# yinyajun/Details-In-Recommendation

Hardware: AMD Instinct MI355X
Metric: CTR samples/sec (embedding gather + FM 2nd-order, 26-field batch 65536) (higher is better)
Workload: dtype f32; 1 GPU; deepfm_gather_fm; batch=65536, fields=26, vocab_per_field=1000000, dim=16, ids=uniform, id_layout=bf, row_policy=auto, parallelism=single GPU, tables resident (1.66 GB)

## Files before the change

### details-in-recommendation_amd/_lib.py

```python
import ctypes
import os

_HERE = os.path.dirname(os.path.abspath(__file__))
_LIB_PATH = os.environ.get("DIR_HIP_LIBRARY") or os.path.join(_HERE, "libdir_hip.so")

c_i32, c_i64, c_f32p, c_vp = ctypes.c_int, ctypes.c_int64, ctypes.c_void_p, ctypes.c_void_p

SIGNATURES = {
    "dir_version": (c_i32, []),
    "dir_last_error": (ctypes.c_char_p, []),
    "dir_crc32c": (ctypes.c_uint32, [ctypes.c_uint32, c_vp, c_i64]),
    "dir_embedding_bag_f32": (c_i32, [c_vp, c_i32, c_i32, c_vp, c_vp, c_vp, c_i64, c_i64, c_i32, c_i32, c_i64,
                                      c_vp, c_i64, c_vp]),
    "dir_embedding_bag_ex_f32": (c_i32, [c_vp, c_vp, c_i32, c_i32, c_vp, c_vp, c_vp, c_i64, c_i64, c_vp, c_i32, ctypes.c_float, c_i32,
                                         c_i64, c_vp, c_i64, c_vp]),
    "dir_embedding_bag_ex2_f32": (c_i32, [c_vp, c_vp, c_i32, c_i32, c_vp, c_vp, c_vp, c_i64, c_i64, c_vp, c_i32, c_vp, ctypes.c_float, c_i32,
                                          c_i64, c_vp, c_i64, c_vp]),
    "dir_check_ids": (c_i32, [c_vp, c_i32, c_vp, c_vp, c_i64, c_i64, c_i64, c_vp, c_vp]),
    "dir_fm_second_order_f32": (c_i32, [c_vp, c_i64, c_i64, c_i32, c_i32, c_vp, c_vp]),
    "dir_linear_onehot_rows_f32": (c_i32, [c_vp, c_i64, c_vp, c_i32, c_vp, c_i64, c_i64, c_vp, c_i32, c_i64, c_vp, c_vp]),
    "dir_sparse_ftrl_rows_sorted_f32": (c_i32, [c_vp, c_i32, c_vp, c_i64, c_i64, c_vp, c_i64, c_i64, ctypes.c_float, ctypes.c_float,
                                                ctypes.c_float, c_i64, c_vp, c_i64, c_vp, c_i64, c_vp, c_vp]),
    "dir_gather_fm_fused_f32": (c_i32, [c_vp, c_vp, c_i32, c_i32, c_vp, c_i64, c_i64, c_i32, c_i64, c_vp, c_i64, c_vp, c_vp]),
    "dir_gather_fm_linear_packed_f32": (c_i32, [c_vp, c_vp, c_i32, c_i32, c_i64, c_i32, c_vp, c_i64, c_i64, c_i32, c_i64, c_vp, c_i64,
                                                c_vp, c_vp, c_vp, c_vp]),
    "dir_gather_fm_rows_f32": (c_i32, [c_vp, c_vp, c_i32, c_i32, c_i64, c_vp, c_i64, c_i64, c_i32, c_i64, c_vp, c_i64, c_vp, c_vp, c_vp]),
    "dir_gather_fm_rows_bits_f32": (c_i32, [c_vp, c_vp, c_i32, c_i32, c_i64, c_vp, c_i64, c_i64, c_i32, c_i64, c_vp, c_i64, c_vp, c_vp, c_vp,
                                            c_vp, c_vp, c_vp]),
    "dir_linear_sparse_sum_f32": (c_i32, [c_vp, c_vp, c_i32, c_vp, c_vp, c_vp, c_i64, c_i64, c_i32, c_vp, c_i32, c_i64,
                                          c_vp, c_vp]),
    "dir_dcn_cross_f32": (c_i32, [c_vp, c_i64, c_vp, c_vp, c_i32, c_i64, c_i32, c_vp, c_i64, c_vp]),
    "dir_dcn_cross_op_f32": (c_i32, [c_vp, c_vp, c_i64, c_vp, c_vp, c_i64, c_i32, c_vp, c_i64, c_vp]),
    "dir_dcn_cross_head_f32": (c_i32, [c_vp, c_i64, c_vp, c_vp, c_i32, c_i64, c_i32, c_vp, c_vp, c_i64, c_vp, c_vp]),
    "dir_fm_second_order_backward_f32": (c_i32, [c_vp, c_i64, c_vp, c_vp, c_i64, c_i64, c_i32, c_i32, c_vp, c_i64, c_vp]),
    "dir_dense_gated_f32": (c_i32, [c_vp, c_i64, c_vp, c_i64, c_vp, c_i64, c_i64, c_i32, c_i32, c_vp, c_i64, c_vp]),
    "dir_dense_dw_bf16x3_workspace_bytes": (c_i64, [c_i64, c_i32, c_i32]),
    "dir_dense_dw_bf16x3_f32": (c_i32, [c_vp, c_i64, c_vp, c_i64, c_i64, c_i32, c_i32, c_vp, c_i64, c_vp, c_vp, c_i64, c_vp]),
    "dir_dense_dw_f16x2_f32": (c_i32, [c_vp, c_i64, c_vp, c_i64, c_i64, c_i32, c_i32, c_vp, c_i64, c_vp, c_vp, c_i64, c_vp, c_vp]),
    "dir_dense_dw_f16x2_scaled_f32": (c_i32, [c_vp, c_i64, c_vp, c_i64, c_i64, c_i32, c_i32, c_vp, c_i64, c_vp, c_vp, c_i64, c_vp, c_vp, c_vp]),
    "dir_row_absmax_workspace_words": (c_i32, []),
    "dir_row_absmax_bits_f32": (c_i32, [c_vp, c_i64, c_i64, c_i32, c_vp, c_vp, c_vp, c_vp]),
    "dir_dense_f16x2_rows_f32": (c_i32, [c_vp, c_i64, c_vp, c_vp, c_i32, c_vp, c_vp, c_vp, c_i64, c_i64, c_i32, c_i32, c_vp, c_i64, c_vp, c_vp, c_vp, c_vp]),
    "dir_dense_dw_small_workspace_bytes": (c_i64, [c_i64, c_i32, c_i32]),
    "dir_dense_dw_small_f32": (c_i32, [c_vp, c_i64, c_vp, c_i64, c_i64, c_i32, c_i32, c_vp, c_i64, c_vp, c_vp, c_i64, c_vp]),
    "dir_units1_relu_backward_partials": (c_i64, [c_i64, c_i32]),
    "dir_units1_relu_backward_f32": (c_i32, [c_vp, c_vp, c_vp, c_i64, c_i64, c_i32, c_vp, c_i64, c_vp, c_i64, c_vp]),
    "dir_units1_relu_backward_bits_f32": (c_i32, [c_vp, c_vp, c_vp, c_i64, c_i64, c_i32, c_vp, c_i64, c_vp, c_i64, c_vp, c_vp, c_vp]),
    "dir_units1_backward_partials": (c_i64, [c_i64, c_i32]),
    "dir_units1_backward_f32": (c_i32, [c_vp, c_vp, c_vp, c_i64, c_i64, c_i32, c_vp, c_i64, c_vp, c_vp, c_i64, c_vp]),
    "dir_units1_f32": (c_i32, [c_vp, c_i64, c_i64, c_i32, c_vp, c_vp, c_vp, c_i64, c_vp]),
    "dir_bn_train_partials": (c_i64, [c_i64, c_i32]),
    "dir_bn_train_stats_f32": (c_i32, [c_vp, c_i64, c_i64, c_i32, ctypes.c_float, ctypes.c_float, c_vp, c_vp, c_vp, c_vp, c_vp, c_vp, c_vp, c_vp, c_vp,
                                       c_i64, c_vp]),
    "dir_bn_train_backward_f32": (c_i32, [c_vp, c_i64, c_vp, c_i64, c_i64, c_i32, c_vp, c_vp, c_vp, c_i32, c_vp, c_i64, c_vp, c_vp, c_vp, c_vp, c_i64,
                                          c_vp]),
    "dir_dice_train_backward_f32": (c_i32, [c_vp, c_i64, c_vp, c_i64, c_i64, c_i32, c_vp, c_vp, c_vp, c_vp, c_vp, c_vp, c_i64, c_vp, c_vp, c_vp, c_i64,
                                            c_vp]),
    "dir_dense_affine_f32": (c_i32, [c_vp, c_i64, c_vp, c_i64, c_vp, c_i32, c_vp, c_vp, c_i64, c_i32, c_i32, c_vp, c_i64, c_vp]),
    "dir_dense_small_f32": (c_i32, [c_vp, c_i64, c_vp, c_i64, c_vp, c_i32, c_vp, c_vp, c_i64, c_i32, c_i32, c_vp, c_i64, c_vp]),
    "dir_dense_mid_f32": (c_i32, [c_vp, c_i64, c_vp, c_i64, c_vp, c_i32, c_vp, c_vp, c_i64, c_i32, c_i32, c_vp, c_i64, c_vp]),
    "dir_tower_bf16x3_image_bytes": (c_i64, [c_i32, c_i32]),
    "dir_tower_bf16x3_pack_f32": (c_i32, [c_vp, c_i64, c_i32, c_i32, c_vp, c_i64, c_vp]),
    "dir_tower_bf16x3_f32": (c_i32, [c_vp, c_i64, c_i64, c_i32, c_i32, c_vp, c_vp, c_vp, c_vp, c_vp, c_vp, c_vp, c_vp, c_vp, c_vp, c_vp, c_i64, c_vp]),
    "dir_deepfm_tower_bf16x3_f32": (c_i32, [c_vp, c_vp, c_i32, c_i32, c_i64, c_i32, c_vp, c_i64, c_i64, c_i32, c_i64, c_vp, c_i32, c_vp, c_vp, c_vp, c_vp,
                                            c_vp, c_vp, c_vp, c_vp, c_vp, c_vp, c_vp, c_i64, c_vp]),
    "dir_tower_f16x2_pack_f32": (c_i32, [c_vp, c_i64, c_i32, c_i32, c_vp, c_i64, c_vp]),
    "dir_tower_f16x2_f32": (c_i32, [c_vp, c_i64, c_i64, c_i32, c_i32, c_vp, c_vp, c_vp, c_vp, c_vp, c_vp, c_vp, c_vp, c_vp, c_vp, c_vp, c_i64, c_vp]),
    "dir_deepfm_tower_f16x2_f32": (c_i32, [c_vp, c_vp, c_i32, c_i32, c_i64, c_i32, c_vp, c_i64, c_i64, c_i32, c_i64, c_vp, c_i32, c_vp, c_vp, c_vp, c_vp,
                                           c_vp, c_vp, c_vp, c_vp, c_vp, c_vp, c_vp, c_i64, c_vp]),
    "dir_esmm_head_f32": (c_i32, [c_vp, c_vp, c_i64, ctypes.c_float, c_vp, c_vp]),
    "dir_tower_cs_image_bytes": (c_i64, [c_i32, c_i32]),
    "dir_tower_cs_f16x2_pack_f32": (c_i32, [c_vp, c_i64, c_i32, c_i32, c_vp, c_i64, c_vp]),
    "dir_tower_cs_f16x2_f32": (c_i32, [c_vp, c_i64, c_i64, c_i32, c_i32, c_vp, c_vp, c_vp, c_vp, c_vp, c_vp, c_vp, c_vp, c_vp, c_vp, c_vp, c_i64, c_vp]),
    "dir_deepfm_tower_cs_f16x2_f32": (c_i32, [c_vp, c_vp, c_i32, c_i32, c_i64, c_i32, c_vp, c_i64, c_i64, c_i32, c_i64, c_vp, c_i32, c_vp, c_vp, c_vp, c_vp,
                                              c_vp, c_vp, c_vp, c_vp, c_vp, c_vp, c_vp, c_i64, c_vp]),
    "dir_dense_f16x2_pack_strided_f32": (c_i32, [c_vp, c_i64, c_i64, c_i32, c_i32, c_vp, c_i64, c_vp]),
# ... 217 lines not shown
```

### details-in-recommendation_amd/csrc/embedding_bag.hip

```cpp
#include "common.hpp"
#include "bag_row.hpp"

namespace dir {

template <int LPS, int VEC, int KT, int UF, bool DO_FM, bool DO_OUT, bool NT>
__global__ __launch_bounds__(256) void gather_onehot_k(const float* const* __restrict__ tables,
                                                       const int64_t* __restrict__ vocab,
                                                       const int64_t* __restrict__ ids, int64_t sb,
                                                       int64_t sf, int F, int Krt, int64_t B,
                                                       float* __restrict__ out, int64_t out_ld,
                                                       float* __restrict__ fm) {
    using V = typename VecT<VEC>::T;
    constexpr int SPW = 64 / LPS;
    const int K = KT > 0 ? KT : Krt;
    const int lane = threadIdx.x & 63;
    const int c = lane & (LPS - 1);
    const int s = lane / LPS;
    const int kv = (K + VEC - 1) / VEC;
    const bool cact = c < kv;
    const int64_t nwave = (int64_t)gridDim.x * (blockDim.x >> 6);
    for (int64_t g = (int64_t)blockIdx.x * (blockDim.x >> 6) + (threadIdx.x >> 6); g * SPW < B; g += nwave) {
        const int64_t b = g * SPW + s;
        const bool act = cact && (b < B);
        const int64_t* idp = ids + (act ? b * sb : 0);
        float* op = DO_OUT ? out + (act ? b * out_ld : 0) + c * VEC : nullptr;
        V sum = vzero((V*)nullptr), sq = vzero((V*)nullptr);
        for (int f0 = 0; f0 < F; f0 += UF) {
            int64_t id[UF];
#pragma unroll
            for (int u = 0; u < UF; ++u) {
                const int f = f0 + u;
                id[u] = (act && f < F) ? idp[(int64_t)f * sf] : (int64_t)-1;
            }
            V row[UF];
#pragma unroll
            for (int u = 0; u < UF; ++u) {
                const int f = f0 + u;
                row[u] = vzero((V*)nullptr);
                if (f < F) {
                    const float* t = tables[f];
                    if ((uint64_t)id[u] < id_bound(vocab, f)) row[u] = NT ? ldv_nt(t + id[u] * K + c * VEC, (V*)nullptr) : ldv(t + id[u] * K + c * VEC, (V*)nullptr);
                }
            }
#pragma unroll
            for (int u = 0; u < UF; ++u) {
                const int f = f0 + u;
                if (f < F) {
                    if (DO_OUT && act) stv(op + (int64_t)f * K, row[u]);
                    if (DO_FM) {
                        sum = vadd(sum, row[u]);
                        sq = vadd(sq, vmul(row[u], row[u]));
                    }
                }
            }
        }
        if (DO_FM) {
            float r = fm_tail<LPS>(sum, sq, lane, c);
            if (c == LPS - 1 && b < B) fm[b] = r;
        }
    }
}

template <int LPS, int UF, bool NT>
__global__ __launch_bounds__(256) void gather_packed_rows_k(const float* const* __restrict__ tables,
                                                            const int64_t* __restrict__ vocab,
                                                            const int64_t* __restrict__ ids, int64_t sb, int64_t sf,
                                                            int F, int K, int64_t ld, int lin_col, int64_t B,
                                                            float* __restrict__ out, int64_t out_ld,
                                                            float* __restrict__ fm, const float* __restrict__ bias,
                                                            float* __restrict__ lin_out,
                                                            float* __restrict__ fsum ,
                                                            unsigned int* __restrict__ row_bits = nullptr ,
                                                            unsigned int* __restrict__ all_bits = nullptr ,
                                                            unsigned int* __restrict__ block_bits = nullptr, unsigned int* __restrict__ ticket = nullptr) {
// ... 184 lines not shown
                                            int K, float* __restrict__ out) {
    using V = typename VecT<VEC>::T;
    constexpr int SPW = 64 / LPS;
    const int lane = threadIdx.x & 63;
    const int c = lane & (LPS - 1);
    const int s = lane / LPS;
    const int kv = (K + VEC - 1) / VEC;
    const bool cact = c < kv;
    const int64_t nwave = (int64_t)gridDim.x * (blockDim.x >> 6);
    for (int64_t g = (int64_t)blockIdx.x * (blockDim.x >> 6) + (threadIdx.x >> 6); g * SPW < B; g += nwave) {
        const int64_t b = g * SPW + s;
        const bool act = cact && (b < B);
        const float* ep = emb + (act ? b * ld : 0) + c * VEC;
        V sum = vzero((V*)nullptr), sq = vzero((V*)nullptr);
#pragma unroll 8
        for (int f = 0; f < F; ++f) {
            V r = act ? ldv(ep + (int64_t)f * K, (V*)nullptr) : vzero((V*)nullptr);
            sum = vadd(sum, r);
            sq = vadd(sq, vmul(r, r));
        }
        float r = fm_tail<LPS>(sum, sq, lane, c);
        if (c == LPS - 1 && b < B) out[b] = r;
    }
}

__global__ void check_ids_k(const int64_t* __restrict__ vocab, int F, const int64_t* __restrict__ ids,
                            const int64_t* __restrict__ offsets, int64_t sb, int64_t sf, int64_t B,
                            int32_t* __restrict__ bad) {
    const int64_t n = B * F;
    int local = 0;
    for (int64_t i = (int64_t)blockIdx.x * blockDim.x + threadIdx.x; i < n; i += (int64_t)gridDim.x * blockDim.x) {
        const int64_t b = i / F;
        const int f = (int)(i - b * F);
        const int64_t v = vocab[f];
        if (!offsets) {
            const int64_t id = ids[b * sb + f * sf];
            if (id >= v || id < -1) ++local;
        } else {
            const int64_t bag = b * sb + f * sf;
            for (int64_t e = offsets[bag]; e < offsets[bag + 1]; ++e)
                if (ids[e] >= v || ids[e] < -1) ++local;
        }
    }
    if (local) atomicAdd(bad, local);
}

static int next_pow2(int v) {
    int p = 1;
    while (p < v) p <<= 1;
    return p;
}

template <int LPS, int VEC, int KT, bool DO_FM, bool DO_OUT>
static void launch_onehot_uf(int uf, bool stream_rows, int64_t work_blocks, hipStream_t st, const float* const* tables,
                             const int64_t* vocab, const int64_t* ids, int64_t sb, int64_t sf, int F, int K, int64_t B, float* out,
                             int64_t out_ld, float* fm) {
    static const int nt_force = dev_env_int("DIR_GATHER_NT", -1);
    const bool nt_env = nt_force >= 0 ? nt_force != 0 : stream_rows;
#define DIR_GO(UF)                                                                                                  \
    do {                                                                                                            \
        if (nt_env) {                                                                                               \
            dim3 grid(grid_resident(work_blocks, resident_blocks(gather_onehot_k<LPS, VEC, KT, UF, DO_FM, DO_OUT, true>))); \
            hipLaunchKernelGGL((gather_onehot_k<LPS, VEC, KT, UF, DO_FM, DO_OUT, true>), grid, dim3(256), 0, st, tables, vocab, ids, sb, sf, F, K, B, out, out_ld, fm); \
        } else {                                                                                                    \
            dim3 grid(grid_resident(work_blocks, resident_blocks(gather_onehot_k<LPS, VEC, KT, UF, DO_FM, DO_OUT, false>))); \
            hipLaunchKernelGGL((gather_onehot_k<LPS, VEC, KT, UF, DO_FM, DO_OUT, false>), grid, dim3(256), 0, st, tables, vocab, ids, sb, sf, F, K, B, out, out_ld, fm); \
        }                                                                                                           \
    } while (0)
    switch (uf) {
        case 4: DIR_GO(4); break;
        case 13: DIR_GO(13); break;
        case 26: DIR_GO(26); break;
        default: DIR_GO(8); break;
    }
#undef DIR_GO
}

template <bool DO_FM, bool DO_OUT>
static int launch_onehot(const float* const* tables, const int64_t* vocab, int F, int K, const int64_t* ids, int64_t sb, int64_t sf,
                         int flags, int64_t B, float* out, int64_t out_ld, float* fm, hipStream_t st) {
    const bool vec = (K % 4 == 0) && (!DO_OUT || (out_ld % 4 == 0 && aligned16(out)));
    static const char* uf_str = runtime_env("DIR_GATHER_UF");
    static const int uf_env = uf_str ? atoi(uf_str) : 0;
    int uf = uf_env > 0 ? uf_env : (F == 26 ? 26 : (F % 13 == 0 ? 13 : (F > 48 ? 26 : 8)));
    const bool stream_rows = (flags & DIR_GATHER_STREAM_ROWS) != 0;
    const int lps = next_pow2(vec ? K / 4 : K);
    if (lps > 64) return fail(DIR_E_UNSUPPORTED, "embedding row of K=%d floats is wider than one wave covers (max %d)", K, vec ? 256 : 64);
    const int spw = 64 / lps;
    const int64_t waves = (B + spw - 1) / spw;
    const int64_t grid = (waves + 3) / 4;
#define DIR_CASE(L, V, KT) launch_onehot_uf<L, V, KT, DO_FM, DO_OUT>(uf, stream_rows, grid, st, tables, vocab, ids, sb, sf, F, K, B, out, out_ld, fm)
    if (vec) {
        switch (lps) {
            case 1: DIR_CASE(1, 4, 4); break;
            case 2: if (K == 8) DIR_CASE(2, 4, 8); else DIR_CASE(2, 4, 0); break;
            case 4: if (K == 16) DIR_CASE(4, 4, 16); else DIR_CASE(4, 4, 0); break;
            case 8: if (K == 32) DIR_CASE(8, 4, 32); else DIR_CASE(8, 4, 0); break;
            case 16: if (K == 64) DIR_CASE(16, 4, 64); else DIR_CASE(16, 4, 0); break;
            case 32: DIR_CASE(32, 4, 0); break;
            default: DIR_CASE(64, 4, 0); break;
        }
    } else {
        switch (lps) {
            case 1: DIR_CASE(1, 1, 1); break;
            case 2: DIR_CASE(2, 1, 0); break;
            case 4: DIR_CASE(4, 1, 0); break;
            case 8: DIR_CASE(8, 1, 0); break;
            case 16: DIR_CASE(16, 1, 0); break;
            case 32: DIR_CASE(32, 1, 0); break;
            default: DIR_CASE(64, 1, 0); break;
        }
    }
#undef DIR_CASE
    DIR_CHECK_LAUNCH("gather_onehot");
    return DIR_OK;
}

static int launch_csr(const float* const* tables, const int64_t* vocab, int F, int K, const int64_t* ids, const int64_t* offsets,
                      const float* weights, int64_t sb, int64_t sf, const int32_t* slot_combiner, int combiner, const float* slot_max_norm,
                      float max_norm, int flags, int64_t B, float* out, int64_t out_ld, hipStream_t st) {
    const bool vec = (K % 4 == 0) && (out_ld % 4 == 0) && aligned16(out);
    const int lps = next_pow2(vec ? K / 4 : K);
    if (lps > 64) return fail(DIR_E_UNSUPPORTED, "embedding row of K=%d floats is wider than one wave covers", K);
    const int spw = 64 / lps;
    const int64_t waves = (B + spw - 1) / spw;
    dim3 grid(grid_for((waves + 3) / 4));
#define DIR_CASE(L, V)                                                                                                              \
    do {                                                                                                                            \
        if (max_norm > 0.f || slot_max_norm)                                                                                        \
            hipLaunchKernelGGL((bag_csr_k<L, V, true>), grid, dim3(256), 0, st, tables, vocab, ids, offsets, weights, sb, sf, F, K, B, \
                               slot_combiner, combiner, slot_max_norm, max_norm, flags, out, out_ld);                               \
        else                                                                                                                        \
            hipLaunchKernelGGL((bag_csr_k<L, V, false>), grid, dim3(256), 0, st, tables, vocab, ids, offsets, weights, sb, sf, F, K, B, \
                               slot_combiner, combiner, slot_max_norm, max_norm, flags, out, out_ld);                               \
    } while (0)
    if (vec) {
        switch (lps) {
            case 1: DIR_CASE(1, 4); break;
            case 2: DIR_CASE(2, 4); break;
            case 4: DIR_CASE(4, 4); break;
            case 8: DIR_CASE(8, 4); break;
            case 16: DIR_CASE(16, 4); break;
            case 32: DIR_CASE(32, 4); break;
            default: DIR_CASE(64, 4); break;
// ... 12 lines not shown
#undef DIR_CASE
    DIR_CHECK_LAUNCH("bag_csr");
    return DIR_OK;
}

}

using namespace dir;

extern "C" int dir_embedding_bag_ex2_f32(const float* const* tables, const int64_t* vocab, int F, int K, const int64_t* ids,
                                         const int64_t* offsets, const float* weights, int64_t stride_b, int64_t stride_f,
                                         const int32_t* slot_combiner, int combiner, const float* slot_max_norm, float max_norm, int flags,
                                         int64_t B, float* out, int64_t out_ld, dir_stream_t stream) {
    DIR_CHECK_ARG(F > 0 && K > 0 && B >= 0, "dir_embedding_bag_f32: F=%d K=%d B=%lld", F, K, (long long)B);
    if (B == 0) return DIR_OK;
    DIR_CHECK_ARG(tables && ids && out, "dir_embedding_bag_f32: null pointer");
    DIR_CHECK_ARG(out_ld >= (int64_t)F * K, "dir_embedding_bag_f32: out_ld=%lld < F*K=%lld", (long long)out_ld, (long long)F * K);
    DIR_CHECK_ARG(combiner >= DIR_COMBINER_SUM && combiner <= DIR_COMBINER_SQRTN, "dir_embedding_bag_f32: combiner=%d", combiner);
    DIR_CHECK_ARG(offsets || !weights, "dir_embedding_bag_f32: weights need offsets (multi-hot)");
    DIR_CHECK_ARG(!(max_norm < 0.f), "dir_embedding_bag_f32: max_norm=%g", max_norm);
    if (!offsets && !(max_norm > 0.f) && !slot_max_norm)
        return launch_onehot<false, true>(tables, vocab, F, K, ids, stride_b, stride_f, flags, B, out, out_ld, nullptr, as_stream(stream));
    return launch_csr(tables, vocab, F, K, ids, offsets, weights, stride_b, stride_f, slot_combiner, combiner, slot_max_norm, max_norm, flags, B,
                      out, out_ld, as_stream(stream));
}

extern "C" int dir_embedding_bag_ex_f32(const float* const* tables, const int64_t* vocab, int F, int K, const int64_t* ids,
                                        const int64_t* offsets, const float* weights, int64_t stride_b, int64_t stride_f,
                                        const int32_t* slot_combiner, int combiner, float max_norm, int flags, int64_t B,
                                        float* out, int64_t out_ld, dir_stream_t stream) {
    return dir_embedding_bag_ex2_f32(tables, vocab, F, K, ids, offsets, weights, stride_b, stride_f, slot_combiner, combiner, nullptr, max_norm,
                                     flags, B, out, out_ld, stream);
}

extern "C" int dir_embedding_bag_f32(const float* const* tables, int F, int K, const int64_t* ids,
                                     const int64_t* offsets, const float* weights, int64_t stride_b,
                                     int64_t stride_f, int combiner, int flags, int64_t B, float* out,
                                     int64_t out_ld, dir_stream_t stream) {
    return dir_embedding_bag_ex_f32(tables, nullptr, F, K, ids, offsets, weights, stride_b, stride_f, nullptr, combiner, 0.f, flags, B,
                                    out, out_ld, stream);
}

extern "C" int dir_gather_fm_fused_f32(const float* const* tables, const int64_t* vocab, int F, int K, const int64_t* ids,
                                       int64_t stride_b, int64_t stride_f, int flags, int64_t B, float* out,
                                       int64_t out_ld, float* fm, dir_stream_t stream) {
    DIR_CHECK_ARG(F > 0 && K > 0 && B >= 0, "dir_gather_fm_fused_f32: F=%d K=%d B=%lld", F, K, (long long)B);
    if (B == 0) return DIR_OK;
    DIR_CHECK_ARG(tables && ids && (out || fm), "dir_gather_fm_fused_f32: null pointer");
    DIR_CHECK_ARG(!out || out_ld >= (int64_t)F * K, "dir_gather_fm_fused_f32: out_ld=%lld < F*K", (long long)out_ld);
    hipStream_t st = as_stream(stream);
    if (out && fm) return launch_onehot<true, true>(tables, vocab, F, K, ids, stride_b, stride_f, flags, B, out, out_ld, fm, st);
    if (fm) return launch_onehot<true, false>(tables, vocab, F, K, ids, stride_b, stride_f, flags, B, nullptr, 0, fm, st);
    return launch_onehot<false, true>(tables, vocab, F, K, ids, stride_b, stride_f, flags, B, out, out_ld, nullptr, st);
}

extern "C" int dir_fm_second_order_f32(const float* emb, int64_t emb_ld, int64_t B, int F, int K, float* out,
                                       dir_stream_t stream) {
    DIR_CHECK_ARG(emb && out, "dir_fm_second_order_f32: null pointer");
    DIR_CHECK_ARG(F > 0 && K > 0 && B >= 0 && emb_ld >= (int64_t)F * K, "dir_fm_second_order_f32: F=%d K=%d B=%lld ld=%lld", F, K, (long long)B, (long long)emb_ld);
    if (B == 0) return DIR_OK;
    const bool vec = (K % 4 == 0) && (emb_ld % 4 == 0) && aligned16(emb);
    const int lps = next_pow2(vec ? K / 4 : K);
    if (lps > 64) return fail(DIR_E_UNSUPPORTED, "dir_fm_second_order_f32: K=%d too wide", K);
    const int spw = 64 / lps;
    const int64_t waves = (B + spw - 1) / spw;
    dim3 grid(grid_for((waves + 3) / 4));
    hipStream_t st = as_stream(stream);
#define DIR_CASE(L, V) hipLaunchKernelGGL((fm_k<L, V>), grid, dim3(256), 0, st, emb, emb_ld, B, F, K, out)
    if (vec) {
        switch (lps) {
            case 1: DIR_CASE(1, 4); break;
            case 2: DIR_CASE(2, 4); break;
            case 4: DIR_CASE(4, 4); break;
            case 8: DIR_CASE(8, 4); break;
            case 16: DIR_CASE(16, 4); break;
            case 32: DIR_CASE(32, 4); break;
            default: DIR_CASE(64, 4); break;
        }
    } else {
        switch (lps) {
            case 1: DIR_CASE(1, 1); break;
            case 2: DIR_CASE(2, 1); break;
            case 4: DIR_CASE(4, 1); break;
            case 8: DIR_CASE(8, 1); break;
            case 16: DIR_CASE(16, 1); break;
            case 32: DIR_CASE(32, 1); break;
            default: DIR_CASE(64, 1); break;
        }
    }
#undef DIR_CASE
    DIR_CHECK_LAUNCH("fm_second_order");
    return DIR_OK;
}

extern "C" int dir_check_ids(const int64_t* vocab, int F, const int64_t* ids, const int64_t* offsets,
                             int64_t stride_b, int64_t stride_f, int64_t B, int32_t* bad_count,
                             dir_stream_t stream) {
    DIR_CHECK_ARG(vocab && ids && bad_count && F > 0 && B >= 0, "dir_check_ids: bad argument");
    hipStream_t st = as_stream(stream);
    if (zero_async(bad_count, sizeof(int32_t), st) != hipSuccess) return fail(DIR_E_HIP, "dir_check_ids: memset failed");
    if (B == 0) return DIR_OK;
    dim3 grid(grid_for((B * F + 255) / 256));
    hipLaunchKernelGGL(check_ids_k, grid, dim3(256), 0, st, vocab, F, ids, offsets, stride_b, stride_f, B, bad_count);
    DIR_CHECK_LAUNCH("check_ids");
    return DIR_OK;
}
// ... 66 lines not shown
```

### details-in-recommendation_amd/ops.py

```python
import ctypes
import os

import torch

from . import _lib
from ._abi import _stream, _dev, _ptr, _onehot_strides
from ._cache import (VersionCache, version_caches, invalidate_caches, capture_hold, frozen_weights, held, capture_guard,
                     capture_bypasses_caches, also_cleared, hip_bumps, mark_written, _CACHE_GEN, _HOLDS, _FROZEN_WEIGHTS)
from .sparse_opt import SparseAdagrad, SparseAdam, SparseFtrl, share_sorted_entries

SUM, MEAN, SQRTN = 0, 1, 2
_COMBINERS = {"sum": SUM, "mean": MEAN, "sqrtn": SQRTN, SUM: SUM, MEAN: MEAN, SQRTN: SQRTN}
PRUNE_NONPOSITIVE_WEIGHTS = 1
STREAM_ROWS = 2
INFINITY_CACHE_BYTES = 256 << 20


class TableSet:

    def __init__(self, tables, ld=None):
        tables = list(tables)
        if not tables:
            raise ValueError("empty columns.")
        K = tables[0].shape[-1] if tables[0].dim() == 2 else 1
        for i, t in enumerate(tables):
            _dev(t, torch.float32, "table %d" % i)
            if ld is None and not t.is_contiguous():
                raise ValueError("table %d must be contiguous" % i)
            if ld is not None and (t.dim() != 2 or tuple(t.stride()) != (ld, 1)):
                raise ValueError("table %d must be a [vocab, K] view with row stride %d" % (i, ld))
            k = t.shape[-1] if t.dim() == 2 else 1
            if k != K:
                raise ValueError("all tables of one TableSet share K (got %d and %d)" % (K, k))
            if (K * 4) % 16 == 0 and t.data_ptr() % 16:
                raise ValueError("table %d is not 16-byte aligned" % i)
        self.tables = tables
        self.F = len(tables)
        self.K = K
        self.vocab = [int(t.shape[0]) for t in tables]
        self.device = tables[0].device
        self.ld = K if ld is None else int(ld)
        self.accums = None
        self._ptrs = torch.tensor([t.data_ptr() for t in tables], dtype=torch.int64, device=self.device)
        self.vocab_dev = torch.tensor(self.vocab, dtype=torch.int64, device=self.device)
        self.row_policy = "auto"
        self.nbytes = sum(int(t.shape[0]) * self.ld * 4 for t in tables)
        self.owners = []
        self.grad_sink = None
        self.fm_sink = None

    @property
    def ptrs(self):
        if self.ld != self.K:
            raise ValueError("this TableSet holds packed training rows (row stride %d, K = %d): only gather_fm and the "
                             "SparseAdagrad update read that layout" % (self.ld, self.K))
        return self._ptrs

    @classmethod
    def train_rows(cls, tables, initial_accumulator_value=0.1):
        tables = list(tables)
        K = int(tables[0].shape[1])
        ld = 2 * K
        vocab = [int(t.shape[0]) for t in tables]
        dev = tables[0].device
        arena = torch.empty(sum(vocab) * ld + 32, dtype=torch.float32, device=dev)
        off = (-(arena.data_ptr() // 4)) % 32
        rows = []
        for t, v in zip(tables, vocab):
            blk = arena[off:off + v * ld].view(v, ld)
            blk[:, :K] = t
            blk[:, K:] = initial_accumulator_value
            rows.append(blk)
            off += v * ld
        ts = cls([r[:, :K] for r in rows], ld=ld)
        ts.accums = [r[:, K:] for r in rows]
        ts.arena, ts.rows = arena, rows
        return ts

    @classmethod
    def ftrl_rows(cls, weights, initial_accumulator_value=0.1):
        weights = [w.reshape(-1, 1) for w in weights]
        vocab = [int(w.shape[0]) for w in weights]
        dev = weights[0].device
        arena = torch.zeros(sum(vocab) * 4 + 4, dtype=torch.float32, device=dev)
        off = (-(arena.data_ptr() // 4)) % 4
        rows = []
        for w, v in zip(weights, vocab):
            blk = arena[off:off + v * 4].view(v, 4)
            blk[:, 0:1] = w
            blk[:, 1] = initial_accumulator_value
            rows.append(blk)
            off += v * 4
        ts = cls([r[:, 0:1] for r in rows], ld=4)
        ts.accums = [r[:, 1:2] for r in rows]
        ts.linears = [r[:, 2:3] for r in rows]
        ts.arena, ts.rows = arena, rows
        return ts

    def absmax(self, every=1):
        watched = list(self.tables) + list(self.owners)
        capture_guard(watched)
        sig = tuple(t._version for t in watched)
        hit = getattr(self, "_absmax", None)
        stale = hit is None or hit[3] != _CACHE_GEN[0] or len(hit[0]) != len(sig)
        if not stale and hit[0] != sig:
            bumps = tuple(hip_bumps(t) for t in watched)
            moved = [v - v0 for v, v0 in zip(sig, hit[0])]
            stale = every <= 1 or any(d != b - b0 or d < 0 or d >= every for d, b, b0 in zip(moved, bumps, hit[2]))
        if stale:
            if self.device.type == "cuda" and torch.cuda.is_current_stream_capturing():
                if hit is not None:
                    return hit[1]
                raise RuntimeError("TableSet.absmax: measure the tables (one eager call) before capturing a graph")
            m = float(torch.stack([t.abs().max() for t in self.tables if t.numel()] or [torch.zeros((), device=self.device)]).max())
            hit = self._absmax = (sig, m, tuple(hip_bumps(t) for t in watched), _CACHE_GEN[0])
        return hit[1]

    def range_ok(self, every=32):
        return f16_range_ok(self.absmax(every))

    def gather_flags(self):
        if self.row_policy == "stream" or (self.row_policy == "auto" and self.nbytes > 2 * INFINITY_CACHE_BYTES):
            return STREAM_ROWS
        return 0

    def written(self, *more):
        arena = getattr(self, "arena", None)
        if arena is not None:
            mark_written(arena, *self.owners, *more)
        else:
            mark_written(*self.tables, *self.owners, *more)

    def refresh(self):
        self._ptrs = torch.tensor([t.data_ptr() for t in self.tables], dtype=torch.int64, device=self.device)



def f16_range_ok(absmax):
    return absmax == 0.0 or (F16_SMALL_GUARD <= absmax < F16_RANGE_GUARD)


class CapturedStep:

    def __init__(self, fn, written=(), warmup=3, pool=None):
        self.fn, self.written = fn, [t for t in written if isinstance(t, torch.Tensor)]
        side = torch.cuda.Stream()
        side.wait_stream(torch.cuda.current_stream())
        with torch.cuda.stream(side):
            for _ in range(max(1, warmup)):
                fn()
        torch.cuda.current_stream().wait_stream(side)
        torch.cuda.synchronize()
        mark_written(*self.written)
        self.graph = torch.cuda.CUDAGraph()
        with capture_hold() as self.hold, torch.cuda.graph(self.graph, pool=pool):
            self.out = fn()
        mark_written(*self.written)

    def replay(self):
        self.graph.replay()
        mark_written(*self.written)
        return self.out


def written_of(*modules_or_tensors):
    out = []
    for m in modules_or_tensors:
        if isinstance(m, torch.Tensor):
            out.append(m)
        else:
            out += list(m.parameters()) + list(m.buffers())
    return out


def refuse_rebuild_under_sink(*tablesets):
    for ts in tablesets:
        if ts is not None and (ts.grad_sink is not None or ts.fm_sink is not None):
# ... 2367 lines not shown
```

### include/dir_hip.h

```cpp
#ifndef DIR_HIP_H_
#define DIR_HIP_H_

#include <stdint.h>

#ifdef __cplusplus
extern "C" {
#endif

typedef void* dir_stream_t;

#define DIR_VERSION 202

enum {
    DIR_OK = 0,
    DIR_E_BADARG = -1,
    DIR_E_RANGE = -2,
    DIR_E_HIP = -3,
    DIR_E_UNSUPPORTED = -4
};

enum { DIR_COMBINER_SUM = 0, DIR_COMBINER_MEAN = 1, DIR_COMBINER_SQRTN = 2 };

enum {
    DIR_BAG_PRUNE_NONPOSITIVE_WEIGHTS = 1,
    DIR_GATHER_STREAM_ROWS = 2
};

int dir_version(void);
const char* dir_last_error(void);

uint32_t dir_crc32c(uint32_t crc, const void* data, int64_t n);

int dir_embedding_bag_f32(const float* const* tables, int F, int K,
                          const int64_t* ids, const int64_t* offsets, const float* weights,
                          int64_t stride_b, int64_t stride_f, int combiner, int flags, int64_t B,
                          float* out, int64_t out_ld, dir_stream_t stream);

int dir_embedding_bag_ex_f32(const float* const* tables, const int64_t* vocab, int F, int K,
                             const int64_t* ids, const int64_t* offsets, const float* weights,
                             int64_t stride_b, int64_t stride_f, const int32_t* slot_combiner, int combiner,
                             float max_norm, int flags, int64_t B, float* out, int64_t out_ld, dir_stream_t stream);

int dir_embedding_bag_ex2_f32(const float* const* tables, const int64_t* vocab, int F, int K,
                              const int64_t* ids, const int64_t* offsets, const float* weights,
                              int64_t stride_b, int64_t stride_f, const int32_t* slot_combiner, int combiner,
                              const float* slot_max_norm, float max_norm, int flags, int64_t B, float* out, int64_t out_ld,
                              dir_stream_t stream);

int dir_check_ids(const int64_t* vocab, int F, const int64_t* ids, const int64_t* offsets,
                  int64_t stride_b, int64_t stride_f, int64_t B, int32_t* bad_count,
                  dir_stream_t stream);

int dir_fm_second_order_f32(const float* emb, int64_t emb_ld, int64_t B, int F, int K, float* out,
                            dir_stream_t stream);

int dir_gather_fm_fused_f32(const float* const* tables, const int64_t* vocab, int F, int K, const int64_t* ids,
                            int64_t stride_b, int64_t stride_f, int flags, int64_t B, float* out,
                            int64_t out_ld, float* fm, dir_stream_t stream);

int dir_gather_fm_linear_packed_f32(const float* const* tables, const int64_t* vocab, int F, int K, int64_t ld, int lin_col,
                                    const int64_t* ids, int64_t stride_b, int64_t stride_f, int flags,
                                    int64_t B, float* out, int64_t out_ld, float* fm, const float* bias,
                                    float* lin_out, dir_stream_t stream);

int dir_gather_fm_rows_f32(const float* const* tables, const int64_t* vocab, int F, int K, int64_t ld, const int64_t* ids,
                           int64_t stride_b, int64_t stride_f, int flags, int64_t B, float* out, int64_t out_ld,
                           float* fm, float* fsum, dir_stream_t stream);
int dir_gather_fm_rows_bits_f32(const float* const* tables, const int64_t* vocab, int F, int K, int64_t ld, const int64_t* ids,
                                int64_t stride_b, int64_t stride_f, int flags, int64_t B, float* out, int64_t out_ld,
                                float* fm, float* fsum, unsigned int* row_bits, unsigned int* all_bits, unsigned int* workspace,
                                dir_stream_t stream);

int dir_linear_sparse_sum_f32(const float* const* weights, const int64_t* vocab, int F, const int64_t* ids,
                              const int64_t* offsets, const float* entry_weights, int64_t stride_b,
                              int64_t stride_f, int combiner, const float* bias, int accumulate,
                              int64_t B, float* out, dir_stream_t stream);

int dir_dcn_cross_f32(const float* x0, int64_t x_ld, const float* w, const float* b, int L,
                      int64_t B, int d, float* out, int64_t out_ld, dir_stream_t stream);

int dir_dcn_cross_op_f32(const float* x0, const float* x, int64_t x_ld, const float* w, const float* b,
                         int64_t B, int d, float* out, int64_t out_ld, dir_stream_t stream);

int dir_dcn_cross_head_f32(const float* x0, int64_t x_ld, const float* w, const float* b, int L, int64_t B, int d,
                           const float* head_w, float* out, int64_t out_ld, float* head_out, dir_stream_t stream);

int dir_din_attention_pool_f32(const float* table, int K, const int64_t* hist,
                               const int32_t* hist_len, const int64_t* cand, int T,
                               const float* W1, const float* b1, int H1, const float* W2,
                               const float* b2, int H2, const float* W3, const float* b3,
                               int normalize, int64_t B, float* out, float* scores,
                               dir_stream_t stream);

enum { DIR_DIN_ACT_SIGMOID = 0, DIR_DIN_ACT_PRELU = 1, DIR_DIN_ACT_DICE = 2 };
int dir_din_activation_rows_f32(float* x, int64_t ld, int64_t B, int N, int activation, const float* alpha, const float* scale,
                                const float* shift, dir_stream_t stream);
int dir_din_attention_pool_act_f32(const float* table, int K, const int64_t* hist, const int32_t* hist_len, const int64_t* cand, int T,
                                   const float* W1, const float* b1, int H1, const float* W2, const float* b2, int H2, const float* W3,
                                   const float* b3, int normalize, int activation, const float* act_params, int64_t B, float* out,
                                   float* scores, dir_stream_t stream);

int dir_cin_layer_f32(const float* x0, const float* xk, const float* W, int m, int Hp, int H, int D,
                      int64_t B, float* xout, float* pooled, int64_t pooled_ld,
                      dir_stream_t stream);
int64_t dir_cin_bf16x3_workspace_bytes(int m, int Hp, int H);
int dir_cin_layer_bf16x3_f32(const float* x0, const float* xk, const float* W, int m, int Hp, int H, int D,
                             int64_t B, float* xout, float* pooled, int64_t pooled_ld,
                             void* workspace, int64_t workspace_bytes, dir_stream_t stream);
int dir_cin_pool_z_f32(const float* x0, const float* xk, int m, int Hp, int D, int64_t B, float* Z, dir_stream_t stream);
int dir_cin_pool_z_bits_f32(const float* x0, const float* xk, int m, int Hp, int D, int64_t B, float* Z, unsigned int* z_row_bits, dir_stream_t stream);
int64_t dir_cin_pooled_image_bytes(int m, int Hp, int H, int D);
// ... 451 lines not shown
```

Measured before the change: 1.054 billion samples/s.

## Add quad-cooperative id loading and branchless row gather path for K=16 one-hot FM

Adds a specialized gather path for K=16 rows where each 4-lane quad loads the sample's ids cooperatively with wide 16-byte loads and spreads them via DPP broadcasts. Table bases and vocab bounds are read once per lane and broadcast with readlane. All row loads are issued up front without branching; out-of-range ids are clamped to row 0 and masked to zero afterwards. It also sets a launch-bounds occupancy hint and adds a tables-nonempty flag that gates the route. The aim is to cut id-load instructions and scalar overhead and to raise memory-level parallelism, at the cost of more register pressure and code complexity.

```diff
diff --git a/details-in-recommendation_amd/_lib.py b/details-in-recommendation_amd/_lib.py
--- a/details-in-recommendation_amd/_lib.py
+++ b/details-in-recommendation_amd/_lib.py
@@ -22,6 +22,7 @@
     "dir_sparse_ftrl_rows_sorted_f32": (c_i32, [c_vp, c_i32, c_vp, c_i64, c_i64, c_vp, c_i64, c_i64, ctypes.c_float, ctypes.c_float,
                                                 ctypes.c_float, c_i64, c_vp, c_i64, c_vp, c_i64, c_vp, c_vp]),
     "dir_gather_fm_fused_f32": (c_i32, [c_vp, c_vp, c_i32, c_i32, c_vp, c_i64, c_i64, c_i32, c_i64, c_vp, c_i64, c_vp, c_vp]),
+    "dir_gather_onehot_route": (c_i32, [c_i32, c_i32, c_i64, c_i64, c_vp, c_i64, c_i32]),
     "dir_gather_fm_linear_packed_f32": (c_i32, [c_vp, c_vp, c_i32, c_i32, c_i64, c_i32, c_vp, c_i64, c_i64, c_i32, c_i64, c_vp, c_i64,
                                                 c_vp, c_vp, c_vp, c_vp]),
     "dir_gather_fm_rows_f32": (c_i32, [c_vp, c_vp, c_i32, c_i32, c_i64, c_vp, c_i64, c_i64, c_i32, c_i64, c_vp, c_i64, c_vp, c_vp, c_vp]),
diff --git a/details-in-recommendation_amd/csrc/embedding_bag.hip b/details-in-recommendation_amd/csrc/embedding_bag.hip
--- a/details-in-recommendation_amd/csrc/embedding_bag.hip
+++ b/details-in-recommendation_amd/csrc/embedding_bag.hip
@@ -3,13 +3,77 @@
 
 namespace dir {
 
-template <int LPS, int VEC, int KT, int UF, bool DO_FM, bool DO_OUT, bool NT>
-__global__ __launch_bounds__(256) void gather_onehot_k(const float* const* __restrict__ tables,
-                                                       const int64_t* __restrict__ vocab,
-                                                       const int64_t* __restrict__ ids, int64_t sb,
-                                                       int64_t sf, int F, int Krt, int64_t B,
-                                                       float* __restrict__ out, int64_t out_ld,
-                                                       float* __restrict__ fm) {
+typedef const char __attribute__((address_space(1))) * gchar_p;
+typedef const f32x4_t __attribute__((address_space(1))) * gf32x4_p;
+typedef int64_t i64x2_a8_t __attribute__((ext_vector_type(2), aligned(8)));
+
+__device__ __forceinline__ int quad_bcast(int v, int q) {
+    switch (q & 3) {
+        case 0: return __builtin_amdgcn_mov_dpp(v, 0x00, 0xf, 0xf, true);
+        case 1: return __builtin_amdgcn_mov_dpp(v, 0x55, 0xf, 0xf, true);
+        case 2: return __builtin_amdgcn_mov_dpp(v, 0xaa, 0xf, 0xf, true);
+        default: return __builtin_amdgcn_mov_dpp(v, 0xff, 0xf, 0xf, true);
+    }
+}
+__device__ __forceinline__ int64_t quad_bcast64(int64_t v, int q) {
+    const unsigned lo = (unsigned)quad_bcast((int)(unsigned)(uint64_t)v, q);
+    const unsigned hi = (unsigned)quad_bcast((int)(unsigned)((uint64_t)v >> 32), q);
+    return (int64_t)(((uint64_t)hi << 32) | lo);
+}
+__device__ __forceinline__ uint64_t lane_u64(uint64_t v, int l) {
+    const unsigned lo = (unsigned)__builtin_amdgcn_readlane((int)(unsigned)v, l);
+    const unsigned hi = (unsigned)__builtin_amdgcn_readlane((int)(unsigned)(v >> 32), l);
+    return ((uint64_t)hi << 32) | lo;
+}
+
+__device__ __forceinline__ float4 keep_if(float4 v, unsigned bit) {
+    const unsigned m = 0u - bit;
+    return make_float4(__uint_as_float(__float_as_uint(v.x) & m), __uint_as_float(__float_as_uint(v.y) & m),
+                       __uint_as_float(__float_as_uint(v.z) & m), __uint_as_float(__float_as_uint(v.w) & m));
+}
+
+template <int UF, bool NT>
+__device__ __forceinline__ unsigned issue_quad_rows(const float* const* __restrict__ tables, const int64_t* __restrict__ vocab,
+                                                    const int64_t* __restrict__ ids_u ,
+                                                    unsigned soff ,
+                                                    int lane, unsigned c16, float4 (&row)[UF]) {
+    static_assert(UF <= 32 && UF % 2 == 0, "one bit per slot; two ids per piece");
+    const unsigned fl = lane < UF ? lane : UF - 1;
+    const uint64_t tb_l = reinterpret_cast<uint64_t>(tables[fl]);
+    const uint64_t bd_v = (uint64_t)(vocab ? vocab : reinterpret_cast<const int64_t*>(tables))[fl];
+    const uint64_t bd_l = vocab ? bd_v : (uint64_t)1 << 63;
+    constexpr int NP = UF / 2, NPL = (NP + 3) / 4;
+    int64_t pc[NPL][2];
+    const gchar_p q = (gchar_p)ids_u + soff;
+#pragma unroll
+    for (int j = 0; j < NPL; ++j) {
+        const int o = (4 * j + 3 < NP || c16 + 64 * j < 16 * NP) ? 64 * j : 16 * (NP - 1) - (int)c16;
+        const i64x2_a8_t v = *reinterpret_cast<const i64x2_a8_t __attribute__((address_space(1)))*>(q + o);
+        pc[j][0] = v.x;
+        pc[j][1] = v.y;
+    }
+    __builtin_amdgcn_sched_barrier(0);
+    unsigned ok = 0u;
+#pragma unroll
+    for (int u = 0; u < UF; ++u) {
+        const int64_t i = quad_bcast64(pc[(u >> 1) >> 2][u & 1], (u >> 1) & 3);
+        const bool in = (uint64_t)i < lane_u64(bd_l, u);
+        ok |= in ? 1u << u : 0u;
+        const gchar_p t = (gchar_p)lane_u64(tb_l, u) + (((in ? i : (int64_t)0) << 6) + c16);
+        const f32x4_t v = NT ? __builtin_nontemporal_load((gf32x4_p)t) : *(gf32x4_p)t;
+        row[u] = make_float4(v.x, v.y, v.z, v.w);
+    }
+    __builtin_amdgcn_sched_barrier(0);
+    return (unsigned)__builtin_amdgcn_mov_dpp((int)ok, 0xe4, 0xf, 0xf, true);
+}
+
+template <int LPS, int VEC, int KT, int UF, bool DO_FM, bool DO_OUT, bool NT, bool QUAD = false>
+__global__ __launch_bounds__(256, (LPS == 4 && VEC == 4 && KT == 16) ? 4 : 1) void gather_onehot_k(const float* const* __restrict__ tables,
+                                                          const int64_t* __restrict__ vocab,
+                                                          const int64_t* __restrict__ ids, int64_t sb,
+                                                          int64_t sf, int F, int Krt, int64_t B,
+                                                          float* __restrict__ out, int64_t out_ld,
+                                                          float* __restrict__ fm) {
     using V = typename VecT<VEC>::T;
     constexpr int SPW = 64 / LPS;
     const int K = KT > 0 ? KT : Krt;
@@ -19,7 +83,38 @@
     const int kv = (K + VEC - 1) / VEC;
     const bool cact = c < kv;
     const int64_t nwave = (int64_t)gridDim.x * (blockDim.x >> 6);
-    for (int64_t g = (int64_t)blockIdx.x * (blockDim.x >> 6) + (threadIdx.x >> 6); g * SPW < B; g += nwave) {
+    const int wv = __builtin_amdgcn_readfirstlane((int)(threadIdx.x >> 6));
+    if constexpr (QUAD) {
+        static_assert(LPS == 4 && VEC == 4 && KT == 16, "issue_quad_rows: quads of 16-byte chunks");
+        for (int64_t g = (int64_t)blockIdx.x * (blockDim.x >> 6) + wv; g * SPW < B; g += nwave) {
+            const int64_t b0 = g * SPW;
+            const int left = B - b0 < SPW ? (int)(B - b0) : SPW;
+            const bool live = s < left;
+            const unsigned sc = live ? s : left - 1;
+            const unsigned c16 = 16u * c;
+            float4 sum = make_float4(0.f, 0.f, 0.f, 0.f), sq = sum;
+            float4 row[UF];
+            const unsigned ok = issue_quad_rows<UF, NT>(tables, vocab, ids + b0 * sb, sc * (unsigned)sb * 8u + c16, lane, c16, row);
+            char* op = DO_OUT ? reinterpret_cast<char*>(out + b0 * out_ld) + ((unsigned)__builtin_amdgcn_mov_dpp((int)sc, 0xe4, 0xf, 0xf, true) * (unsigned)out_ld * 4u + c16) : nullptr;
+            if (live) {
+#pragma unroll
+                for (int u = 0; u < UF; ++u) {
+                    row[u] = keep_if(row[u], (ok >> u) & 1u);
+                    if (DO_OUT) stv(reinterpret_cast<float*>(op + u * KT * 4), row[u]);
+                    if (DO_FM) {
+                        sum = vadd(sum, row[u]);
+                        sq = vadd(sq, vmul(row[u], row[u]));
+                    }
+                }
+            }
+            if (DO_FM) {
+                float r = fm_tail<LPS>(sum, sq, lane, c);
+                if (c == LPS - 1 && live) fm[b0 + s] = r;
+            }
+        }
+        return;
+    }
+    for (int64_t g = (int64_t)blockIdx.x * (blockDim.x >> 6) + wv; g * SPW < B; g += nwave) {
         const int64_t b = g * SPW + s;
         const bool act = cact && (b < B);
         const int64_t* idp = ids + (act ? b * sb : 0);
@@ -310,44 +405,55 @@
 }
 
 template <int LPS, int VEC, int KT, bool DO_FM, bool DO_OUT>
-static void launch_onehot_uf(int uf, bool stream_rows, int64_t work_blocks, hipStream_t st, const float* const* tables,
+static void launch_onehot_uf(int uf, bool stream_rows, bool quad, int64_t work_blocks, hipStream_t st, const float* const* tables,
                              const int64_t* vocab, const int64_t* ids, int64_t sb, int64_t sf, int F, int K, int64_t B, float* out,
                              int64_t out_ld, float* fm) {
     static const int nt_force = dev_env_int("DIR_GATHER_NT", -1);
     const bool nt_env = nt_force >= 0 ? nt_force != 0 : stream_rows;
-#define DIR_GO(UF)                                                                                                  \
-    do {                                                                                                            \
-        if (nt_env) {                                                                                               \
-            dim3 grid(grid_resident(work_blocks, resident_blocks(gather_onehot_k<LPS, VEC, KT, UF, DO_FM, DO_OUT, true>))); \
-            hipLaunchKernelGGL((gather_onehot_k<LPS, VEC, KT, UF, DO_FM, DO_OUT, true>), grid, dim3(256), 0, st, tables, vocab, ids, sb, sf, F, K, B, out, out_ld, fm); \
-        } else {                                                                                                    \
-            dim3 grid(grid_resident(work_blocks, resident_blocks(gather_onehot_k<LPS, VEC, KT, UF, DO_FM, DO_OUT, false>))); \
-            hipLaunchKernelGGL((gather_onehot_k<LPS, VEC, KT, UF, DO_FM, DO_OUT, false>), grid, dim3(256), 0, st, tables, vocab, ids, sb, sf, F, K, B, out, out_ld, fm); \
-        }                                                                                                           \
-    } while (0)
+    auto go = [&](auto kernel) {
+        dim3 grid(grid_resident(work_blocks, resident_blocks(kernel)));
+        hipLaunchKernelGGL(kernel, grid, dim3(256), 0, st, tables, vocab, ids, sb, sf, F, K, B, out, out_ld, fm);
+    };
+    auto by_uf = [&](auto ufc) {
+        constexpr int UF = decltype(ufc)::value;
+        if constexpr (LPS == 4 && VEC == 4 && KT == 16 && UF % 2 == 0)
+            if (quad) return nt_env ? go(gather_onehot_k<LPS, VEC, KT, UF, DO_FM, DO_OUT, true, true>) : go(gather_onehot_k<LPS, VEC, KT, UF, DO_FM, DO_OUT, false, true>);
+        return nt_env ? go(gather_onehot_k<LPS, VEC, KT, UF, DO_FM, DO_OUT, true>) : go(gather_onehot_k<LPS, VEC, KT, UF, DO_FM, DO_OUT, false>);
+    };
     switch (uf) {
-        case 4: DIR_GO(4); break;
-        case 13: DIR_GO(13); break;
-        case 26: DIR_GO(26); break;
-        default: DIR_GO(8); break;
-    }
-#undef DIR_GO
+        case 4: by_uf(std::integral_constant<int, 4>{}); break;
+        case 13: by_uf(std::integral_constant<int, 13>{}); break;
+        case 26: by_uf(std::integral_constant<int, 26>{}); break;
+        default: by_uf(std::integral_constant<int, 8>{}); break;
+    }
+}
+
+static int onehot_uf(int F) {
+    static const char* uf_str = runtime_env("DIR_GATHER_UF");
+    static const int uf_env = uf_str ? atoi(uf_str) : 0;
+    return uf_env > 0 ? uf_env : (F == 26 ? 26 : (F % 13 == 0 ? 13 : (F > 48 ? 26 : 8)));
+}
+
+static bool onehot_quad_route(int F, int K, int64_t sb, int64_t sf, const float* out, int64_t out_ld, int flags) {
+    const int uf = onehot_uf(F), uf_run = (uf == 4 || uf == 13 || uf == 26) ? uf : 8;
+    const bool vec = !out || (out_ld % 4 == 0 && aligned16(out));
+    return K == 16 && vec && (flags & DIR_GATHER_TABLES_NONEMPTY) && sf == 1 && F == uf_run && F % 2 == 0 && sb >= F && sb < (1 << 24) &&
+           (!out || out_ld < (1 << 24));
 }
 
 template <bool DO_FM, bool DO_OUT>
 static int launch_onehot(const float* const* tables, const int64_t* vocab, int F, int K, const int64_t* ids, int64_t sb, int64_t sf,
                          int flags, int64_t B, float* out, int64_t out_ld, float* fm, hipStream_t st) {
     const bool vec = (K % 4 == 0) && (!DO_OUT || (out_ld % 4 == 0 && aligned16(out)));
-    static const char* uf_str = runtime_env("DIR_GATHER_UF");
-    static const int uf_env = uf_str ? atoi(uf_str) : 0;
-    int uf = uf_env > 0 ? uf_env : (F == 26 ? 26 : (F % 13 == 0 ? 13 : (F > 48 ? 26 : 8)));
+    const int uf = onehot_uf(F);
     const bool stream_rows = (flags & DIR_GATHER_STREAM_ROWS) != 0;
     const int lps = next_pow2(vec ? K / 4 : K);
     if (lps > 64) return fail(DIR_E_UNSUPPORTED, "embedding row of K=%d floats is wider than one wave covers (max %d)", K, vec ? 256 : 64);
     const int spw = 64 / lps;
     const int64_t waves = (B + spw - 1) / spw;
     const int64_t grid = (waves + 3) / 4;
-#define DIR_CASE(L, V, KT) launch_onehot_uf<L, V, KT, DO_FM, DO_OUT>(uf, stream_rows, grid, st, tables, vocab, ids, sb, sf, F, K, B, out, out_ld, fm)
+    const bool quad = onehot_quad_route(F, K, sb, sf, DO_OUT ? out : nullptr, out_ld, flags);
+#define DIR_CASE(L, V, KT) launch_onehot_uf<L, V, KT, DO_FM, DO_OUT>(uf, stream_rows, quad, grid, st, tables, vocab, ids, sb, sf, F, K, B, out, out_ld, fm)
     if (vec) {
         switch (lps) {
             case 1: DIR_CASE(1, 4, 4); break;
@@ -466,6 +572,10 @@
     if (out && fm) return launch_onehot<true, true>(tables, vocab, F, K, ids, stride_b, stride_f, flags, B, out, out_ld, fm, st);
     if (fm) return launch_onehot<true, false>(tables, vocab, F, K, ids, stride_b, stride_f, flags, B, nullptr, 0, fm, st);
     return launch_onehot<false, true>(tables, vocab, F, K, ids, stride_b, stride_f, flags, B, out, out_ld, nullptr, st);
+}
+
+extern "C" int dir_gather_onehot_route(int F, int K, int64_t stride_b, int64_t stride_f, const float* out, int64_t out_ld, int flags) {
+    return onehot_quad_route(F, K, stride_b, stride_f, out, out_ld, flags) ? 1 : 0;
 }
 
 extern "C" int dir_fm_second_order_f32(const float* emb, int64_t emb_ld, int64_t B, int F, int K, float* out,
diff --git a/details-in-recommendation_amd/ops.py b/details-in-recommendation_amd/ops.py
--- a/details-in-recommendation_amd/ops.py
+++ b/details-in-recommendation_amd/ops.py
@@ -13,6 +13,7 @@
 _COMBINERS = {"sum": SUM, "mean": MEAN, "sqrtn": SQRTN, SUM: SUM, MEAN: MEAN, SQRTN: SQRTN}
 PRUNE_NONPOSITIVE_WEIGHTS = 1
 STREAM_ROWS = 2
+TABLES_NONEMPTY = 8
 INFINITY_CACHE_BYTES = 256 << 20
 
 
@@ -38,6 +39,7 @@
         self.F = len(tables)
         self.K = K
         self.vocab = [int(t.shape[0]) for t in tables]
+        self._nonempty = min(self.vocab) > 0
         self.device = tables[0].device
         self.ld = K if ld is None else int(ld)
         self.accums = None
@@ -120,9 +122,10 @@
         return f16_range_ok(self.absmax(every))
 
     def gather_flags(self):
+        flags = TABLES_NONEMPTY if self._nonempty else 0
         if self.row_policy == "stream" or (self.row_policy == "auto" and self.nbytes > 2 * INFINITY_CACHE_BYTES):
-            return STREAM_ROWS
-        return 0
+            flags |= STREAM_ROWS
+        return flags
 
     def written(self, *more):
         arena = getattr(self, "arena", None)
diff --git a/include/dir_hip.h b/include/dir_hip.h
--- a/include/dir_hip.h
+++ b/include/dir_hip.h
@@ -23,7 +23,8 @@
 
 enum {
     DIR_BAG_PRUNE_NONPOSITIVE_WEIGHTS = 1,
-    DIR_GATHER_STREAM_ROWS = 2
+    DIR_GATHER_STREAM_ROWS = 2,
+    DIR_GATHER_TABLES_NONEMPTY = 8
 };
 
 int dir_version(void);
@@ -57,6 +58,8 @@
 int dir_gather_fm_fused_f32(const float* const* tables, const int64_t* vocab, int F, int K, const int64_t* ids,
                             int64_t stride_b, int64_t stride_f, int flags, int64_t B, float* out,
                             int64_t out_ld, float* fm, dir_stream_t stream);
+
+int dir_gather_onehot_route(int F, int K, int64_t stride_b, int64_t stride_f, const float* out, int64_t out_ld, int flags);
 
 int dir_gather_fm_linear_packed_f32(const float* const* tables, const int64_t* vocab, int F, int K, int64_t ld, int lin_col,
                                     const int64_t* ids, int64_t stride_b, int64_t stride_f, int flags,
```

Result: faster. 1.142 billion samples/s (median of 6 runs) (+8.4%).
